# liuyuan-pal/NeuRay

Measured on AMD Instinct MI355X. Metric: rays/sec (64 coarse+32 fine samples), lego 800x800 synthetic, higher is better.
Workload: dtype fp32 (MLP contractions: operands split exactly into 3 bf16 parts, 6 bf16-MFMA products per K = 32, fp32 accumulate); 1 GPU; lego-800 synthetic (nerf_synthetic/lego/black_800 shape): 800x800 = 640000 rays/image, 8 ref views, 64 coarse + 32 fine samples, maps 200x200x32, 1 image per step per GPU; ray_batch=65536, parallelism=images sharded over 1 GPU(s), no collective

## Files before the change

### neuray_amd/csrc/nr_kernels.h

```cpp
#pragma once
#include "nr_device.h"

namespace nr {

__global__ void view_setup_kernel(const float* __restrict__ poses, const float* __restrict__ Ks,
                                  const float* __restrict__ depth_range, int n, float* __restrict__ out) {
    const int v = blockIdx.x * blockDim.x + threadIdx.x;
    if (v >= n) return;
    const float* P = poses + v * 12;
    const float* K = Ks + v * 9;
    float* o = out + v * kViewConst;
    for (int i = 0; i < 3; ++i)
        for (int j = 0; j < 4; ++j)
            o[i * 4 + j] = dot3(K[i * 3 + 0], K[i * 3 + 1], K[i * 3 + 2], P[j], P[4 + j], P[8 + j]);
    for (int i = 0; i < 3; ++i) o[12 + i] = dot3(-P[i], -P[4 + i], -P[8 + i], P[3], P[7], P[11]);
    o[15] = rn_div(-1.0f, depth_range[2 * v]);
    o[16] = rn_div(-1.0f, depth_range[2 * v + 1]);
    o[17] = rn_div(1.0f, rn_sub(o[16], o[15]));
    o[18] = 0.0f; o[19] = 0.0f;
}

__global__ void query_setup_kernel(const float* __restrict__ pose, const float* __restrict__ Kinv,
                                   const float* __restrict__ depth_range, float* __restrict__ o) {
    if (blockIdx.x * blockDim.x + threadIdx.x != 0) return;
    for (int i = 0; i < 9; ++i) o[i] = Kinv[i];
    for (int i = 0; i < 12; ++i) o[9 + i] = pose[i];
    for (int i = 0; i < 3; ++i) o[21 + i] = dot3(-pose[i], -pose[4 + i], -pose[8 + i], pose[3], pose[7], pose[11]);
    o[24] = rn_div(-1.0f, depth_range[0]);
    o[25] = rn_div(-1.0f, depth_range[1]);
    o[26] = depth_range[0];
    o[27] = rn_div(1.0f, rn_sub(o[25], o[24]));
}

__global__ void relayout_kernel(const float* __restrict__ src, float* __restrict__ dst, int n, int c, int h, int w, int c_pad) {
    const long long total = (long long)n * h * w;
    for (long long i = (long long)blockIdx.x * blockDim.x + threadIdx.x; i < total; i += (long long)gridDim.x * blockDim.x) {
        const long long img = i / ((long long)h * w);
        const long long pix = i - img * h * w;
        const float* s = src + img * c * h * w + pix;
        float* d = dst + i * c_pad;
        for (int ch = 0; ch < c_pad; ++ch) d[ch] = ch < c ? s[(long long)ch * h * w] : 0.0f;
    }
}

__global__ void coarse_depth_kernel(const float* __restrict__ depth_range, const float* __restrict__ rnd, int rn, int dn,
                                    float* __restrict__ out) {
    const float near = depth_range[0], far = depth_range[1];
    const long long total = (long long)rn * dn;
    for (long long i = (long long)blockIdx.x * blockDim.x + threadIdx.x; i < total; i += (long long)gridDim.x * blockDim.x) {
        const int k = (int)(i % dn);
        if (rnd && k > 0 && k < dn - 1) {
            const float inv_near = rn_div(1.0f, near);
            const float step = rn_div(rn_sub(rn_div(1.0f, far), inv_near), (float)(dn - 1));
            const float val = rn_add((float)k, rn_mul(rn_sub(rnd[(i / dn) * (dn - 2) + (k - 1)], 0.5f), 0.999f));
            out[i] = rn_div(1.0f, rn_add(inv_near, rn_mul(step, val)));
        } else {
            out[i] = coarse_depth(near, far, k, dn);
        }
    }
}

struct PointParams {
    const float* que_const;
    const float* view_const;
    const float* coords;
    const float* depth;
    const float* ray_feats;
    const float* img_feats;
    const float* rgba;
    const float* weights;
    float* point_out;
    float* dbg;
    float* saved;
    int rfn, rn, dn, h, w, fh, fw;
    int use_vis;
    float var_bias;
    int folded;
    unsigned long long* slot_stats;
};

constexpr int kDbgFields = 16;

constexpr int kSavedBgRow = 0, kSavedStatRow = 16, kSavedMsumRow = 60, kSavedSw0Row = 61, kSavedGeoRow = 62, kSavedGmeanRow = 78,
              kSavedGvarRow = 86, kSavedGRow = 94, kSavedZmaxRow = 98, kSavedSezRow = 99, kSavedSvisRow = 100, kSavedDist = 101 * 64;
constexpr int kSavedTileFloats = kSavedDist + 8 * 8 * 16;

__device__ __forceinline__ float sel4(int g, float a, float b, float c, float d) {
    return g == 0 ? a : (g == 1 ? b : (g == 2 ? c : d));
}

template <int NT>
constexpr int point_rmax() { return 12 * NT; }

template <int NT>
inline size_t point_smem_bytes(int nwaves, int ar = AR_F32) {
    return sizeof(float) * (64 * ((size_t)(nwaves + 1) * point_rmax<NT>() + (ar == AR_X3 ? 0 : 16 * NT)) + weight_lds_floats(ar));
}

template <int NT, int OWN, int STAT, class WS>
__device__ __forceinline__ void bg_accumulate(WS W, int lane, int g, int wave, int nw,
                                              const float (&st)[NT * 11], v4f (&accg)[OWN][NT]) {
    float xq[NT][8], x1[NT][1];
    NR_PRAGMA_UNROLL
    for (int t = 0; t < NT; ++t) {
        NR_PRAGMA_UNROLL
        for (int s = 0; s < 8; ++s) xq[t][s] = st[t * 11 + s];
        x1[t][0] = sel4(g, st[t * 11 + 8], st[t * 11 + 9], st[t * 11 + 10], 0.0f);
    }
    NR_PRAGMA_UNROLL
    for (int j = 0; j < OWN; ++j) {
        const int mo = wave + j * nw;
        if (mo < 4) layer_tile_slice<L_BG, NT, 2 * STAT, 2, STAT, 1>(W, lane, mo, xq, x1, accg[j]);
    }
}

template <int OWN> struct BgResident { float4 q[OWN][8]; float s1[OWN][4]; float4 b[OWN]; };
template <int OWN, class WS>
__device__ __forceinline__ void bg_resident_load(WS W, int lane, int wave, int nw, BgResident<OWN>& r) {
    constexpr int AR = ws_ar<WS>::value;
    NR_PRAGMA_UNROLL
    for (int j = 0; j < OWN; ++j) {
        const int mo = wave + j * nw, m = mo < 4 ? mo : 0;
        NR_PRAGMA_UNROLL
        for (int kq = 0; kq < 8; ++kq) r.q[j][kq] = wld4(W, lane * 16 + m * (8 * 1024), (quads_offset(L_BG, AR) + kq * 256) * 4);
        NR_PRAGMA_UNROLL
        for (int k1 = 0; k1 < 4; ++k1) r.s1[j][k1] = wld1(W, lane * 4 + m * (4 * 256), (single_offset(L_BG, AR) + k1 * 64) * 4);
        r.b[j] = wld4(W, (lane >> 4) * 16 + m * 64, bias_offset(L_BG, AR) * 4);
    }
}
template <int NT, int OWN, int STAT>
__device__ __forceinline__ void bg_accumulate(const BgResident<OWN>& r, int g, int wave, int nw,
                                              const float (&st)[NT * 11], v4f (&accg)[OWN][NT]) {
    float xq[NT][8], x1[NT][1];
    NR_PRAGMA_UNROLL
    for (int t = 0; t < NT; ++t) {
        NR_PRAGMA_UNROLL
        for (int s = 0; s < 8; ++s) xq[t][s] = st[t * 11 + s];
        x1[t][0] = sel4(g, st[t * 11 + 8], st[t * 11 + 9], st[t * 11 + 10], 0.0f);
    }
    NR_PRAGMA_UNROLL
    for (int j = 0; j < OWN; ++j) {
        const int mo = wave + j * nw;
        if (mo < 4) {
            mfma_quad<NT>(r.q[j][2 * STAT], 0, xq, accg[j]);
            mfma_quad<NT>(r.q[j][2 * STAT + 1], 1, xq, accg[j]);
            NR_PRAGMA_UNROLL
            for (int t = 0; t < NT; ++t) accg[j][t] = nr_mfma16(r.s1[j][STAT], x1[t][0], accg[j][t]);
        }
    }
}

template <int NA, int IDLE, int R, int RMAX, int OP>
__device__ __forceinline__ void view_allreduce(const float (&v)[NA > 0 ? NA : 1][R], float (&out)[R], float* red, int wave,
                                               int nw, int lane) {
    NR_PRAGMA_UNROLL
    for (int r = 0; r < R; ++r) {
        const bool is_max = OP == RED_MAX || (OP == RED_MAX0 && r == 0);
        float a = NA > 0 ? v[0][r] : (is_max ? -1e9f : 0.0f);
        NR_PRAGMA_UNROLL
        for (int s = 1; s < NA; ++s) a = red_combine<OP, R>(a, v[s][r], r);
        if (IDLE > 0 && NA > 0 && is_max) a = fmaxf(a, -1e9f);
        out[r] = a;
    }
    block_allreduce<R, RMAX, OP, R>(out, red, wave, nw, lane);
}

template <int N> struct SlotCount { static constexpr int value = N; };

#ifndef NR_POINT_SKIP
#define NR_POINT_SKIP 1
#endif
#ifndef NR_POINT_TILE_ORDER
#define NR_POINT_TILE_ORDER 0
#endif
#ifndef NR_POINT_TRANSPOSED
#define NR_POINT_TRANSPOSED 1
#endif

template <int NT, int VPW, bool HAS_VIS, int OWN, int MAXT, int MINW, bool SAVE = false, bool DBG = false, int AR = AR_F32>
__global__ void __launch_bounds__(MAXT, MINW) points_kernel(PointParams p) {
    static_assert(NT == 1, "one 16-point tile per wave iteration");
    static_assert(AR == AR_F32 || !SAVE, "the training forward runs on the fp32 MFMA");
    NR_DYNAMIC_SMEM(float, smem);
    constexpr int RMAX = point_rmax<NT>();
    constexpr int NS = VPW;
    constexpr bool SKIP = (NR_POINT_SKIP != 0) && !SAVE && !DBG && VPW == 2;
    const int lane = threadIdx.x & 63;
    const int wave = NR_UNIFORM((int)(threadIdx.x >> 6));
    const int nw = (p.rfn + VPW - 1) / VPW;
    const int g = lane >> 4, c = lane & 15;
    float* red = smem;
    float* xch = smem + (size_t)(nw + 1) * RMAX * 64;
    float* wl = xch + (AR == AR_X3 ? 0 : 16 * NT * 64);
    auto xrow = [&](int mo, int r) -> float* {
        if constexpr (AR == AR_X3 && OWN == 1) return red + ((size_t)mo * RMAX + r) * 64;
        else if constexpr (AR == AR_X3) return red + ((size_t)(mo % nw) * RMAX + (mo / nw) * 4 + r) * 64;
        else return xch + (mo * 4 + r) * 64;
    };
    auto make_w = [&]() {
        if constexpr (AR == AR_X3) return GlbW3{nr_make_wbuf(p.weights, sizeof(float) * kPackedPointFloatsX3)};
        else return nr_make_wbuf(p.weights, sizeof(float) * kPackedPassFloats);
    };
    const auto W = make_w();
    const float w_m1 = (float)(p.w - 1), h_m1 = (float)(p.h - 1);
    const float inv_w_m1 = 1.0f / w_m1, inv_h_m1 = 1.0f / h_m1, inv_rfn = 1.0f / (float)p.rfn;
    const size_t fmap = (size_t)p.fh * p.fw * 32, imap = (size_t)p.h * p.w * 4;
    const nr_mbuf rf_map = nr_make_mbuf(p.ray_feats, sizeof(float) * fmap * p.rfn);
    const nr_mbuf if_map = nr_make_mbuf(p.img_feats, sizeof(float) * fmap * p.rfn);
    const nr_mbuf rgb_map = nr_make_mbuf(p.rgba, sizeof(float) * imap * p.rfn);
    const int goff = 32 * g;
    const int npts = p.rn * p.dn;
    const int dn = p.dn;
    const bool use_vis = p.use_vis != 0;
    const bool folded = AR == AR_X3 || (!SAVE && p.folded != 0);
    const int bid = (int)(blockIdx.x % 8) * (int)(gridDim.x / 8) + (int)(blockIdx.x / 8);
    int seq0 = 0;
#ifndef NR_X3_BG_RESIDENT
#define NR_X3_BG_RESIDENT 1
#endif
#ifndef NR_X3_GF_PREFETCH
#define NR_X3_GF_PREFETCH 1
#endif
    constexpr bool BG_RES = AR == AR_X3 && OWN == 1 && (NR_X3_BG_RESIDENT != 0);
    BgResident<OWN> bgres;
    if constexpr (BG_RES) bg_resident_load(W, lane, wave, nw, bgres);
    int n_active = 0, n_slots = 0;
    constexpr bool TR = (NR_POINT_TRANSPOSED != 0) && !SAVE && !DBG;
    const int nloop = TR ? ((p.rn + 15) / 16) * dn * 16 : npts;
#ifndef NR_POINT_CHUNK
#define NR_POINT_CHUNK 1
#endif
    constexpr int CH = NR_POINT_CHUNK;
    const int G = (int)gridDim.x;
    auto tile_base = [&](int it) { return (((it / CH) * G + bid) * CH + (it % CH)) * 16; };
    if (tile_base(0) < nloop) stage_issue<PH_DIST_M>(wl, W, wave, nw, lane);
    for (int it = 0, base; (base = tile_base(it)) < nloop; ++it, seq0 += phase_count(HAS_VIS)) {
        const bool more = tile_base(it + 1) < nloop;
        const int glane = lane + nr_opaque_zero();
#ifndef NR_NO_OPAQUE_WAVE
        const int wave_t = wave + nr_opaque_szero();
#else
        const int wave_t = wave;
#endif
        const int gg = glane >> 4;
        const bool dbg_lane = DBG && (gg == 0);
        const auto* pt = NR_ARGS_HERE(PointParams, p);
        int pidx; bool pvalid;
        float mask[NS], dlt[NS][4], tref[NS], pu[NS], pv[NS], lo, hi;
        int soff_f[NS], soff_c[NS];
        {
            int pi, ray, smp;
            const float* __restrict__ qc = pt->que_const;
            const float qnearp = qc[24], qfarp = qc[25], qinv = qc[27];
            const int dn = pt->dn, npts = pt->rn * dn;
            if constexpr (TR) {
#if NR_POINT_TILE_ORDER == 1
                const int tix = base >> 4, nrb = (pt->rn + 15) / 16;
                smp = tix / nrb;
                const int rb = tix - smp * nrb;
#else
                const int tix = base >> 4, rb = tix / dn;
                smp = tix - rb * dn;
#endif
                ray = rb * 16 + c;
                pvalid = ray < pt->rn;
                ray = pvalid ? ray : pt->rn - 1;
                pi = ray * dn + smp;
            } else {
                pi = base + c;
                pvalid = pi < npts;
                pi = pi < npts ? pi : npts - 1;
                ray = pi / dn;
                smp = pi - ray * dn;
            }
            pidx = pi;
            const Ray r = make_ray<false>(qc, pt->coords[2 * ray], pt->coords[2 * ray + 1]);
            const float* drow = pt->depth + (size_t)ray * dn;
            const float d = drow[smp];
            float s_c, s_n, s_p, s_x;
            {
                const int nxt = smp + 1 < dn ? smp + 1 : smp, prv = smp > 0 ? smp - 1 : 0;
                const float dg = drow[gg == 0 ? smp : (gg == 1 ? nxt : prv)];
                nr_group_gather4(norm_inv_depth_fast(dg, qnearp, qfarp, qinv), s_c, s_n, s_p, s_x);
            }
            const float half_c = (smp == dn - 1) ? 500000.0f : (s_n - s_c) * 0.5f;
            const float half_p = (s_c - s_p) * 0.5f;
            hi = half_c;
            lo = (smp == 0) ? half_c : half_p;
            const float px = rn_add(r.cx, rn_mul(r.dx, d));
            const float py = rn_add(r.cy, rn_mul(r.dy, d));
            const float pz = rn_add(r.cz, rn_mul(r.dz, d));
            NR_PRAGMA_UNROLL
            for (int s = 0; s < NS; ++s) {
                const int vraw = wave_t * VPW + s;
                const bool vok = vraw < pt->rfn;
                const int view = vok ? vraw : pt->rfn - 1;
                const float* __restrict__ vc = pt->view_const + view * kViewConst;
                Proj pr = project_point<false>(vc, px, py, pz, (float)pt->w, (float)pt->h);
                if (!vok) pr.mask = 0.0f;
                mask[s] = pr.mask;
                dlt[s][0] = pr.dirx - r.qx; dlt[s][1] = pr.diry - r.qy; dlt[s][2] = pr.dirz - r.qz;
                dlt[s][3] = dot3(pr.dirx, pr.diry, pr.dirz, r.qx, r.qy, r.qz);
                tref[s] = norm_inv_depth_fast(fmaxf(pr.z, 1e-5f), vc[15], vc[16], vc[17]);
                pu[s] = pr.u; pv[s] = pr.v;
                if (dbg_lane && pvalid && vok) {
                    float* d_ = pt->dbg + ((size_t)pi * pt->rfn + view) * kDbgFields;
                    d_[0] = pr.mask; d_[1] = pr.u; d_[2] = pr.v; d_[3] = pr.z;
                }
                soff_f[s] = view * (int)(fmap * sizeof(float)); soff_c[s] = view * (int)(imap * sizeof(float));
            }
        }

        auto tile = [&](auto na_tag) NR_LAMBDA_INLINE {
            constexpr int NA = decltype(na_tag)::value, NA1 = NA > 0 ? NA : 1, IDLE = NS - NA;
            constexpr bool SC = NA == 2 && !SAVE;
            float fray[NA1][8], fimg[NA1][8], rgb[NA1][3];
#ifdef NR_PROBE_PRE
            float fm1[NA1][8], fv1[NA1][8], fa1[NA1][8];
#endif
            if constexpr (NA > 0) {
                Taps tfs[NA], tcs[NA];
                NR_PRAGMA_UNROLL
                for (int s = 0; s < NA; ++s) {
                    tfs[s] = make_taps_fast(pu[s], pv[s], w_m1, h_m1, inv_w_m1, inv_h_m1, p.fw, p.fh, p.fw == p.w && p.fh == p.h);
                    tcs[s] = make_taps_fast(pu[s], pv[s], w_m1, h_m1, inv_w_m1, inv_h_m1, p.w, p.h, true);
#ifdef NR_PROBE_NO_GATHER
                    tfs[s].o00 = tfs[s].o10 = tfs[s].o01 = tfs[s].o11 = 0;
                    tcs[s].o00 = tcs[s].o10 = tcs[s].o01 = tcs[s].o11 = 0;
#endif
                }
                NR_PRAGMA_UNROLL
                for (int s = 0; s < NA; ++s) {
                    float4 qf[8], qi[8], qc4[4];
                    issue8(rf_map, goff, soff_f[s], tfs[s], qf);
                    issue8(if_map, goff, soff_f[s], tfs[s], qi);
                    issue_rgb(rgb_map, soff_c[s], tcs[s], qc4);
                    NR_PIN();
                    blend8(qf, tfs[s], mask[s], fray[s]);
                    blend8(qi, tfs[s], mask[s], fimg[s]);
                    blend_rgb(qc4, tcs[s], mask[s], rgb[s]);
                    NR_PRAGMA_UNROLL
                    for (int k = 0; k < 8; ++k) { NR_KEEP(fray[s][k]); NR_KEEP(fimg[s][k]); }
                    NR_PRAGMA_UNROLL
                    for (int j = 0; j < 3; ++j) NR_KEEP(rgb[s][j]);
                    NR_PIN();
#ifdef NR_PROBE_PRE
                    {
                        float4 q1[8], q2[8], q3[8];
                        issue8(rf_map, goff, soff_f[s] + 4096, tfs[s], q1);
                        issue8(rf_map, goff, soff_f[s] + 8192, tfs[s], q2);
                        issue8(rf_map, goff, soff_f[s] + 12288, tfs[s], q3);
                        NR_PIN();
                        blend8(q1, tfs[s], mask[s], fm1[s]);
                        blend8(q2, tfs[s], mask[s], fv1[s]);
                        blend8(q3, tfs[s], mask[s], fa1[s]);
                        NR_PRAGMA_UNROLL
                        for (int k = 0; k < 8; ++k) { NR_KEEP(fm1[s][k]); NR_KEEP(fv1[s][k]); NR_KEEP(fa1[s][k]); }
                        NR_PIN();
                    }
#endif
                }
            }
            float none[NA1][1];
            NR_PRAGMA_UNROLL
            for (int s = 0; s < NA1; ++s) none[s][0] = 0.0f;
// ... 215 lines not shown
                        p12[s][11] = mask[s];
                    }
                    view_allreduce<NA, IDLE, 12, RMAX, RED_SUM>(p12, o12, red, wave_t, nw, lane);
                    msum = o12[11];
                    const float inv = nr_fast_rcp(msum + 1e-8f);
                    NR_PRAGMA_UNROLL
                    for (int q = 0; q < 11; ++q) st[q] = o12[q] * inv;
                    NR_PRAGMA_UNROLL
                    for (int s = 0; s < NA; ++s) wv[s] = mask[s] * nr_fast_rcp(msum + 1e-8f);
                    if constexpr (SAVE) {
                        if (wave_t == 0) p.saved[(size_t)(base / 16) * kSavedTileFloats + kSavedMsumRow * 64 + lane] = msum;
                    }
                }
                NR_PRAGMA_UNROLL
                for (int k = 0; k < 2; ++k) {
                    NR_PRAGMA_UNROLL
                    for (int s = 0; s < NA; ++s) wk[s] = k == 0 ? sn[s] * wv[s] : wv[s];
                    if (k == 1) {
                        NR_PRAGMA_UNROLL
                        for (int s = 0; s < NA; ++s) {
                            NR_PRAGMA_UNROLL
                            for (int q = 0; q < 8; ++q) part[s][q] = gi[s][q] * wk[s];
                            NR_PRAGMA_UNROLL
                            for (int j = 0; j < 3; ++j) part[s][8 + j] = gr[s][j] * wk[s];
                        }
                        view_allreduce<NA, IDLE, 11, RMAX, RED_SUM>(part, st, red, wave_t, nw, lane);
                    }
                    NR_PRAGMA_UNROLL
                    for (int s = 0; s < NA; ++s) {
                        NR_PRAGMA_UNROLL
                        for (int q = 0; q < 8; ++q) { const float d_ = gi[s][q] - st[q]; part[s][q] = wk[s] * (d_ * d_); }
                        NR_PRAGMA_UNROLL
                        for (int j = 0; j < 3; ++j) { const float d_ = gr[s][j] - st[8 + j]; part[s][8 + j] = wk[s] * (d_ * d_); }
                    }
                    if constexpr (BG_RES) {
                        if (k == 0) bg_accumulate<NT, OWN, 0>(bgres, gg, wave_t, nw, st, accg);
                        else bg_accumulate<NT, OWN, 2>(bgres, gg, wave_t, nw, st, accg);
                    } else {
                        if (k == 0) bg_accumulate<NT, OWN, 0>(W, glane, gg, wave_t, nw, st, accg);
                        else bg_accumulate<NT, OWN, 2>(W, glane, gg, wave_t, nw, st, accg);
                    }
                    view_allreduce<NA, IDLE, 11, RMAX, RED_SUM>(part, sv, red, wave_t, nw, lane);
                    if constexpr (BG_RES) {
                        if (k == 0) bg_accumulate<NT, OWN, 1>(bgres, gg, wave_t, nw, sv, accg);
                        else bg_accumulate<NT, OWN, 3>(bgres, gg, wave_t, nw, sv, accg);
                    } else {
                        if (k == 0) bg_accumulate<NT, OWN, 1>(W, glane, gg, wave_t, nw, sv, accg);
                        else bg_accumulate<NT, OWN, 3>(W, glane, gg, wave_t, nw, sv, accg);
                    }
                    if constexpr (SAVE) {
                        float* d_ = p.saved + (size_t)(base / 16) * kSavedTileFloats + (kSavedStatRow + 22 * k) * 64 + lane;
                        if (wave_t == (2 * k) % nw) {
                            NR_PRAGMA_UNROLL
                            for (int q = 0; q < 11; ++q) d_[q * 64] = st[q];
                        }
                        if (wave_t == (2 * k + 1) % nw) {
                            NR_PRAGMA_UNROLL
                            for (int q = 0; q < 11; ++q) d_[(11 + q) * 64] = sv[q];
                        }
                    }
                }
                NR_PRAGMA_UNROLL
                for (int j = 0; j < OWN; ++j) {
                    const int mo = wave_t + j * nw;
                    if (mo < 4) {
                        NR_PRAGMA_UNROLL
                        for (int r = 0; r < 4; ++r) xrow(mo, r)[lane] = accg[j][0][r];
                        if constexpr (SAVE) {
                            NR_PRAGMA_UNROLL
                            for (int r = 0; r < 4; ++r)
                                p.saved[(size_t)(base / 16) * kSavedTileFloats + (kSavedBgRow + mo * 4 + r) * 64 + lane] = accg[j][0][r];
                        }
                    }
                }
                NR_BLOCK_SYNC();
                NR_PRAGMA_UNROLL
                for (int s = 0; s < NA; ++s)
                    NR_PRAGMA_UNROLL
                    for (int mo = 0; mo < (AR == AR_X3 ? 2 : 4); ++mo)
                        NR_PRAGMA_UNROLL
                        for (int r = 0; r < 4; ++r) accv[s][mo][r] = xrow(mo, r)[lane];
            }
            float x[NA1][8], vis2[NA1], z[NA1];
            constexpr bool GF_PRE = BG_RES && (NR_X3_GF_PREFETCH != 0);
            float4 gfq[4]; float gfs = 0.0f;
            typename ws_lds<decltype(make_w())>::type W5;
            LayerPreT<L_VF1, AR> p_vf1;
            {
                float xq[NA1][16], x1[NA1][1], h64[NA1][16];
                Opnd3<NA1, 16> xq3;
                LayerPreT<L_BV0, AR> p_bv0; LayerPreT<L_BV1, AR> p_bv1; LayerPreT<L_B2, AR> p_b2;
                v4f acch[NA1][2];
                if constexpr (NA > 0) {
                    NR_PRAGMA_UNROLL
                    for (int s = 0; s < NA; ++s) {
                        NR_PRAGMA_UNROLL
                        for (int k = 0; k < 8; ++k) { xq[s][k] = gi[s][k]; xq[s][8 + k] = e[s][k]; }
                        x1[s][0] = sel4(gg, gr[s][0], gr[s][1], gr[s][2], 0.0f);
                    }
                    layer_prefetch<L_BV0>(W4, lane, p_bv0);
                    NR_PRAGMA_UNROLL
                    for (int s = 0; s < NA; ++s) { acch[s][0] = accv[s][0]; acch[s][1] = accv[s][1]; }
                    if constexpr (AR == AR_X3) {
                        const Opnd3<NA1, 8> gi3 = split_operand(gi);
                        NR_PRAGMA_UNROLL
                        for (int pt = 0; pt < 3; ++pt)
                            NR_PRAGMA_UNROLL
                            for (int s = 0; s < NA; ++s)
                                NR_PRAGMA_UNROLL
                                for (int i = 0; i < 4; ++i) { xq3.p[pt][s][i] = gi3.p[pt][s][i]; xq3.p[pt][s][4 + i] = e3.p[pt][s][i]; }
                        layer_acc<L_BV0, NA>(W4, lane, p_bv0, xq3, x1, acch, last);
                    } else layer_acc<L_BV0, NA>(W4, lane, p_bv0, xq, x1, acch, last);
                    NR_PRAGMA_UNROLL
                    for (int s = 0; s < NA; ++s)
                        NR_PRAGMA_UNROLL
                        for (int mo = 0; mo < 2; ++mo)
                            NR_PRAGMA_UNROLL
                            for (int r = 0; r < 4; ++r) h64[s][4 * mo + r] = elu_s(acch[s][mo][r]);
                }
                const auto W4b = phase_enter<PH_BV1, HAS_VIS>(wl, W, seq0, true, wave_t, nw, lane);
                if constexpr (NA > 0) {
                    layer_prefetch<L_BV1>(W4b, lane, p_bv1);
                    NR_PRAGMA_UNROLL
                    for (int s = 0; s < NA; ++s) {
                        if constexpr (AR == AR_X3) {
                            NR_PRAGMA_UNROLL
                            for (int mo = 0; mo < 2; ++mo)
                                NR_PRAGMA_UNROLL
                                for (int r = 0; r < 4; ++r) acch[s][mo][r] = xrow(2 + mo, r)[lane];
                        } else { acch[s][0] = accv[s][2]; acch[s][1] = accv[s][3]; }
                    }
                    if constexpr (AR == AR_X3) layer_acc<L_BV1, NA>(W4b, lane, p_bv1, xq3, x1, acch, last);
                    else layer_acc<L_BV1, NA>(W4b, lane, p_bv1, xq, x1, acch, last);
                    NR_PRAGMA_UNROLL
                    for (int s = 0; s < NA; ++s)
                        NR_PRAGMA_UNROLL
                        for (int mo = 0; mo < 2; ++mo)
                            NR_PRAGMA_UNROLL
                            for (int r = 0; r < 4; ++r) h64[s][8 + 4 * mo + r] = elu_s(acch[s][mo][r]);
                }
                W5 = phase_enter<PH_B2_VF1, HAS_VIS>(wl, W, seq0, true, wave_t, nw, lane);
                if constexpr (NA > 0) {
                    layer_prefetch<L_B2>(W5, lane, p_b2);
                    layer_fwd<L_B2, NA, ACT_ELU>(W5, lane, p_b2, operand<AR>(h64), none, x, p_vf1);
                }
            }
            {
                float xin[NA1][8], h[NA1][8];
                if constexpr (NA > 0) {
                    NR_PRAGMA_UNROLL
                    for (int s = 0; s < NA; ++s)
                        NR_PRAGMA_UNROLL
                        for (int k = 0; k < 8; ++k) xin[s][k] = x[s][k] * wv[s];
                    layer_fwd<L_VF1, NA, ACT_ELU>(W5, lane, p_vf1, operand<AR>(xin), none, h, last);
                }
                W5 = phase_enter<PH_TAIL, HAS_VIS>(wl, W, seq0, more, wave_t, nw, lane);
                if constexpr (GF_PRE) {
                    const int m = wave_t < 4 ? wave_t : 0;
                    NR_PRAGMA_UNROLL
                    for (int kq = 0; kq < 4; ++kq) gfq[kq] = wld4(W, glane * 16 + m * (4 * 1024), (quads_offset(L_GF1, AR) + kq * 256) * 4);
                    gfs = wld1(W, glane * 4 + m * 256, single_offset(L_GF1, AR) * 4);
                }
                if constexpr (NA > 0) {
                    float y[NA][8], yv[NA][1], o[NA][1];
                    LayerPreT<L_VF2, AR> p_vf2; LayerPreT<L_V21, AR> p_v21; LayerPreT<L_RF1, AR> p_rf1; LayerPreT<L_RF2, AR> p_rf2;
                    VecPre<L_VF2> p_vf2v; VecPre<L_V22> p_v22; VecPre<L_RF3> p_rf3;
                    layer_prefetch<L_VF2>(W5, lane, p_vf2);
                    layer_prefetch<L_VF2>(W5, lane, p_vf2v);
                    layer_fwd<L_VF2, NA, ACT_ELU>(W5, lane, p_vf2, operand<AR>(h), none, y, p_v21);
                    if constexpr (SC) nr_group_gather2(sigmoidf(elu(layer_vec_scatter_1x2<L_VF2, 0>(p_vf2v, h))), yv[0][0], yv[1][0]);
                    else {
                        layer_vec<L_VF2, NA>(p_vf2v, h, yv);
                        NR_PRAGMA_UNROLL
                        for (int s = 0; s < NA; ++s) yv[s][0] = sigmoidf(elu(yv[s][0]));
                    }
                    float visp[NA];
                    NR_PRAGMA_UNROLL
                    for (int s = 0; s < NA; ++s) {
                        visp[s] = yv[s][0] * mask[s];
                        NR_PRAGMA_UNROLL
                        for (int k = 0; k < 8; ++k) { x[s][k] = x[s][k] + y[s][k]; xin[s][k] = x[s][k] * visp[s]; }
                    }
                    Opnd3<NA, 8> x3;
                    if constexpr (AR == AR_X3) {
                        x3 = split_operand(x);
                        layer_fwd_scaled<L_V21, NA, ACT_ELU>(W5, lane, p_v21, x3, visp, h, p_v22);
                    } else layer_fwd<L_V21, NA, ACT_ELU>(W5, lane, p_v21, xin, none, h, p_v22);
                    layer_prefetch<L_RF1>(W5, lane, p_rf1);
                    if constexpr (SC) nr_group_gather2(sigmoidf(layer_vec_scatter_1x2<L_V22, 0>(p_v22, h)), o[0][0], o[1][0]);
                    else {
                        layer_vec<L_V22, NA>(p_v22, h, o);
                        NR_PRAGMA_UNROLL
                        for (int s = 0; s < NA; ++s) o[s][0] = sigmoidf(o[s][0]);
                    }
                    NR_PRAGMA_UNROLL
                    for (int s = 0; s < NA; ++s) vis2[s] = o[s][0] * mask[s];
                    float x1[NA][2], h16[NA][4], h8[NA][4];
                    NR_PRAGMA_UNROLL
                    for (int s = 0; s < NA; ++s) {
                        x1[s][0] = sel4(gg, vis2[s], dlt[s][0], dlt[s][1], dlt[s][2]);
                        x1[s][1] = sel4(gg, dlt[s][3], 0.0f, 0.0f, 0.0f);
                    }
                    if constexpr (AR == AR_X3) layer_fwd<L_RF1, NA, ACT_ELU>(W5, lane, p_rf1, x3, x1, h16, p_rf2);
                    else layer_fwd<L_RF1, NA, ACT_ELU>(W5, lane, p_rf1, x, x1, h16, p_rf2);
                    layer_fwd<L_RF2, NA, ACT_ELU>(W5, lane, p_rf2, operand<AR>(h16), none, h8, p_rf3);
                    if constexpr (SC) nr_group_gather2(layer_vec_scatter_1x2<L_RF3, 0>(p_rf3, h8), o[0][0], o[1][0]);
                    else layer_vec<L_RF3, NA>(p_rf3, h8, o);
                    NR_PRAGMA_UNROLL
                    for (int s = 0; s < NA; ++s) {
                        z[s] = mask[s] > 0.0f ? o[s][0] : -1e9f;
                        const int vraw = wave_t * VPW + s;
                        if (dbg_lane && pvalid && vraw < p.rfn) {
                            float* d_ = pt->dbg + ((size_t)pidx * pt->rfn + vraw) * kDbgFields;
                            d_[12] = sn[s]; d_[13] = visp[s]; d_[14] = vis2[s]; d_[15] = z[s];
                        }
                    }
                }
            }
            constexpr int ZR = SAVE ? 3 : 2;
            float zv[ZR], big[12], wh[NA1], meanw;
            {
                float z2[NA1][ZR];
                NR_PRAGMA_UNROLL
                for (int s = 0; s < NA; ++s) {
                    z2[s][0] = z[s]; z2[s][1] = vis2[s];
                    if constexpr (SAVE) z2[s][2] = sn[s] * wv[s];
                }
                view_allreduce<NA, IDLE, ZR, RMAX, RED_MAX0>(z2, zv, red, wave_t, nw, lane);
                float b12[NA1][12];
                NR_PRAGMA_UNROLL
                for (int s = 0; s < NA; ++s) {
                    const float ev = nr_fast_exp(z[s] - zv[0]);
                    wh[s] = vis2[s] * nr_fast_rcp(zv[1] + 1e-8f);
                    NR_PRAGMA_UNROLL
                    for (int k = 0; k < 8; ++k) b12[s][k] = x[s][k] * wh[s];
                    b12[s][8] = ev;
                    NR_PRAGMA_UNROLL
                    for (int j = 0; j < 3; ++j) b12[s][9 + j] = rgb[s][j] * ev;
                }
                if constexpr (IDLE > 0) {
                    const float ev_idle = nr_fast_exp(-1e9f - zv[0]);
                    if constexpr (NA == 0) {
                        NR_PRAGMA_UNROLL
                        for (int q = 0; q < 12; ++q) b12[0][q] = 0.0f;
                        float acc_ = ev_idle;
                        NR_PRAGMA_UNROLL
                        for (int i = 1; i < IDLE; ++i) acc_ += ev_idle;
                        b12[0][8] = acc_;
                        view_allreduce<1, 0, 12, RMAX, RED_SUM>(b12, big, red, wave_t, nw, lane);
                    } else {
                        NR_PRAGMA_UNROLL
                        for (int i = 0; i < IDLE; ++i) b12[NA - 1][8] += ev_idle;
                        view_allreduce<NA, 0, 12, RMAX, RED_SUM>(b12, big, red, wave_t, nw, lane);
                    }
                } else {
                    view_allreduce<NA, 0, 12, RMAX, RED_SUM>(b12, big, red, wave_t, nw, lane);
                }
                {
                    const float ie = nr_fast_rcp(big[8]);
                    big[9] *= ie; big[10] *= ie; big[11] *= ie;
                    meanw = zv[1] * nr_fast_rcp(zv[1] + 1e-8f);
                }
                if constexpr (SAVE) {
                    float* d_ = p.saved + (size_t)(base / 16) * kSavedTileFloats + lane;
                    if (wave_t == 0) {
                        NR_PRAGMA_UNROLL
                        for (int k = 0; k < 8; ++k) d_[(kSavedGmeanRow + k) * 64] = big[k];
                    }
                    if (wave_t == 2 % nw) {
                        d_[kSavedZmaxRow * 64] = zv[0]; d_[kSavedSezRow * 64] = big[8];
                        d_[kSavedSvisRow * 64] = zv[1]; d_[kSavedSw0Row * 64] = zv[ZR - 1];
                    }
                }
            }
            v4f accf[OWN][1];
            NR_PRAGMA_UNROLL
            for (int j = 0; j < OWN; ++j) {
                const int mo = wave_t + j * nw;
                const float4 b = wld4(W, gg * 16 + (mo < 4 ? mo : 0) * 64, bias_offset(L_GF1, AR) * 4);
                accf[j][0][0] = b.x; accf[j][0][1] = b.y; accf[j][0][2] = b.z; accf[j][0][3] = b.w;
            }
            float var[8];
            {
                float xq[1][8], x1[1][1], v8[NA1][8];
                NR_PRAGMA_UNROLL
                for (int s = 0; s < NA; ++s)
                    NR_PRAGMA_UNROLL
                    for (int k = 0; k < 8; ++k) { const float d_ = x[s][k] - big[k]; v8[s][k] = wh[s] * (d_ * d_); }
                NR_PRAGMA_UNROLL
                for (int k = 0; k < 8; ++k) xq[0][k] = big[k];
                x1[0][0] = sel4(gg, meanw * inv_rfn, 0.0f, 0.0f, 0.0f);
                NR_PRAGMA_UNROLL
                for (int j = 0; j < OWN; ++j) {
                    const int mo = wave_t + j * nw;
                    if constexpr (GF_PRE) {
                        if (mo < 4) {
                            mfma_quad<NT>(gfq[0], 0, xq, accf[j]);
                            mfma_quad<NT>(gfq[1], 1, xq, accf[j]);
                            accf[j][0] = nr_mfma16(gfs, x1[0][0], accf[j][0]);
                        }
                    } else if (mo < 4) layer_tile_slice<L_GF1, NT, 0, 2, 0, 1>(W, glane, mo, xq, x1, accf[j]);
                }
                view_allreduce<NA, IDLE, 8, RMAX, RED_SUM>(v8, var, red, wave_t, nw, lane);
                if constexpr (SAVE) {
                    if (wave_t == 1 % nw) {
                        NR_PRAGMA_UNROLL
                        for (int k = 0; k < 8; ++k) p.saved[(size_t)(base / 16) * kSavedTileFloats + (kSavedGvarRow + k) * 64 + lane] = var[k];
                    }
                }
            }
            {
                float xq[1][8], nonet[1][1];
                nonet[0][0] = 0.0f;
                NR_PRAGMA_UNROLL
                for (int k = 0; k < 8; ++k) xq[0][k] = var[k];
                NR_PRAGMA_UNROLL
                for (int j = 0; j < OWN; ++j) {
                    const int mo = wave_t + j * nw;
                    if (mo < 4) {
                        if constexpr (GF_PRE) { mfma_quad<NT>(gfq[2], 0, xq, accf[j]); mfma_quad<NT>(gfq[3], 1, xq, accf[j]); }
                        else layer_tile_slice<L_GF1, NT, 2, 2, 0, 0>(W, glane, mo, xq, nonet, accf[j]);
                        NR_PRAGMA_UNROLL
                        for (int r = 0; r < 4; ++r) xrow(mo, r)[lane] = elu_s(accf[j][0][r]);
                        if constexpr (SAVE) {
                            NR_PRAGMA_UNROLL
                            for (int r = 0; r < 4; ++r)
                                p.saved[(size_t)(base / 16) * kSavedTileFloats + (kSavedGeoRow + mo * 4 + r) * 64 + lane] = elu_s(accf[j][0][r]);
                        }
                    }
                }
            }
            NR_BLOCK_SYNC();
            if (wave_t == 0) {
                float h[1][16], G[1][4], nonet[1][1];
                nonet[0][0] = 0.0f;
                NR_PRAGMA_UNROLL
                for (int k = 0; k < 16; ++k) h[0][k] = xrow(k >> 2, k & 3)[lane];
                layer_fwd<L_GF2, NT, ACT_ELU>(W, glane, h, nonet, G);
                if (pvalid)
                    *reinterpret_cast<float4*>(pt->point_out + (size_t)pidx * kPointRec + 4 * g) = make_float4(G[0][0], G[0][1], G[0][2], G[0][3]);
                if constexpr (SAVE) {
                    NR_PRAGMA_UNROLL
                    for (int r = 0; r < 4; ++r) p.saved[(size_t)(base / 16) * kSavedTileFloats + (kSavedGRow + r) * 64 + lane] = G[0][r];
                }
            }
            if (wave_t == (nw > 1 ? 1 : 0) && gg == 0) {
                if (pvalid)
                    *reinterpret_cast<float4*>(pt->point_out + (size_t)pidx * kPointRec + 16) = make_float4(big[9], big[10], big[11], msum);
            }
        };

        if constexpr (SKIP) {
            const bool a0 = __ballot(mask[0] != 0.0f) != 0ull, a1 = __ballot(mask[1] != 0.0f) != 0ull;
#ifdef NR_FORCE_NA
#ifdef NR_FORCE_NA_CONST
            const int na = NR_FORCE_NA;
#else
            const int na = NR_FORCE_NA + (p.rn < 0 ? (a0 ? 1 : 0) + (a1 ? 1 : 0) : 0);
#endif
#else
            const int na = (a0 ? 1 : 0) + (a1 ? 1 : 0);
#endif
            n_active += na; n_slots += NS;
            if (na == 2) {
                tile(SlotCount<2>{});
            } else if (na == 1) {
                if (!a0) {
                    mask[0] = mask[1]; tref[0] = tref[1]; pu[0] = pu[1]; pv[0] = pv[1]; soff_f[0] = soff_f[1]; soff_c[0] = soff_c[1];
                    NR_PRAGMA_UNROLL
                    for (int k = 0; k < 4; ++k) dlt[0][k] = dlt[1][k];
                }
                tile(SlotCount<1>{});
            } else {
                tile(SlotCount<0>{});
            }
        } else {
            tile(SlotCount<NS>{});
        }
    }
    if constexpr (SKIP) {
        if (p.slot_stats) {
            NR_BLOCK_SYNC();
            if (lane == 0) { red[2 * wave] = (float)n_active; red[2 * wave + 1] = (float)n_slots; }
            NR_BLOCK_SYNC();
            if (threadIdx.x == 0) {
                float a = 0.0f, b = 0.0f;
                for (int w = 0; w < nw; ++w) { a += red[2 * w]; b += red[2 * w + 1]; }
                atomicAdd(p.slot_stats, (unsigned long long)a);
                atomicAdd(p.slot_stats + 1, (unsigned long long)b);
            }
        }
    }
}

struct RayParams {
    const float* point_rec;
    const float* depth;
    const float* pos_enc;
    const float* weights;
    float* hit_prob;
    float* pixel;
    float* render_depth;
    unsigned char* ray_mask;
    float* density;
    float* att_save;
    int rn, dn, mask_view_num, mask_point_num;
};
constexpr int kRayAttSave = 24;

constexpr int kRayWaves = 4;
inline size_t ray_smem_bytes(int dn, int rays_per_wave = 1) { return sizeof(float) * (kPackedRayFloats + 12 + kRayWaves * rays_per_wave * ((size_t)dn * 34)); }

__device__ __forceinline__ float wave_sum(float v) {
    NR_PRAGMA_UNROLL
    for (int m = 32; m >= 1; m >>= 1) v += __shfl_xor(v, m);
    return v;
}

__device__ __forceinline__ float wave_max(float v) {
    NR_PRAGMA_UNROLL
    for (int m = 32; m >= 1; m >>= 1) v = fmaxf(v, __shfl_xor(v, m));
// ... 685 lines not shown
```

### neuray_amd/csrc/nr_layout.h

```cpp
#pragma once

namespace nr {

enum LayerId {
    L_DM1, L_DM2,
    L_DFIN_M,
    L_DV1, L_DV2,
    L_DFIN_V,
    L_DA1, L_DA2,
    L_DFIN_A,
    L_DS1, L_DS2,
    L_DFIN_S,
    L_PE1, L_PE2,
    L_RD1, L_RD2,
    L_NF1, L_NF2,
    L_BV0, L_BV1,
    L_B2,
    L_VF1, L_VF2,
    L_V21, L_V22,
    L_RF1, L_RF2, L_RF3,
    L_BG,
    L_GF1, L_GF2,
    L_FWD_COUNT,
    LT_DM1 = L_FWD_COUNT, LT_DM2, LT_DV1, LT_DV2, LT_DA1, LT_DA2, LT_DS1, LT_DS2,
// ... 57 lines not shown
};

struct VecShape { int n, tiles; };
constexpr VecShape kVec[L_COUNT] = {
    {0, 0}, {0, 0}, {2, 2},
    {0, 0}, {0, 0}, {2, 2},
    {0, 0}, {0, 0}, {1, 2},
    {0, 0}, {0, 0}, {1, 2},
    {0, 0}, {0, 0},
    {0, 0}, {3, 1},
    {0, 0}, {1, 1},
    {0, 0}, {0, 0}, {0, 0},
    {0, 0}, {1, 2},
    {0, 0}, {1, 2},
    {0, 0}, {0, 0}, {1, 1},
    {0, 0},
    {0, 0}, {0, 0},
    {0, 0}, {0, 0}, {0, 0}, {0, 0}, {0, 0}, {0, 0}, {0, 0}, {0, 0},
    {2, 2}, {0, 0},
    {0, 0},
    {0, 0},
    {3, 4},
    {0, 0},
    {0, 0},
    {3, 4}, {3, 4}, {3, 4}, {3, 4},
    {0, 0}, {0, 0},
    {0, 0},
    {1, 1}, {0, 0},
    {1, 4}, {0, 0},
};

constexpr int AR_F32 = 0, AR_X3 = 1;
constexpr bool ar_omits(int l, int ar) { return ar == AR_X3 && l == L_PE2; }
constexpr bool ar_splits(int l, int ar) { return ar == AR_X3 && l != L_BG && l != L_GF1 && l != L_GF2; }

constexpr int quads_floats(int l, int ar = AR_F32) { return ar_omits(l, ar) ? 0 : kShape[l].mt_out * kShape[l].kq * 64 * (ar_splits(l, ar) ? 6 : 4); }
constexpr int single_floats(int l, int ar = AR_F32) { return ar_omits(l, ar) ? 0 : kShape[l].mt_out * kShape[l].k1 * 64; }
constexpr int bias_floats(int l, int ar = AR_F32) { return ar_omits(l, ar) ? 0 : kShape[l].mt_out * 16; }
constexpr int vec_floats(int l, int ar = AR_F32) { return (kVec[l].n > 0 && !ar_omits(l, ar)) ? kVec[l].n * kVec[l].tiles * 16 + 16 : 0; }
constexpr int layer_floats(int l, int ar = AR_F32) { return quads_floats(l, ar) + single_floats(l, ar) + bias_floats(l, ar) + vec_floats(l, ar); }
constexpr int tile_quads_floats(int l, int ar = AR_F32) { return kShape[l].kq * 64 * (ar_splits(l, ar) ? 6 : 4); }

constexpr int layer_offset(int l, int ar = AR_F32) {
    int off = 0;
    for (int i = (l >= L_FWD_COUNT ? (int)L_FWD_COUNT : 0); i < l; ++i) off += layer_floats(i, ar);
    return off;
}
constexpr int quads_offset(int l, int ar = AR_F32) { return layer_offset(l, ar); }
constexpr int single_offset(int l, int ar = AR_F32) { return layer_offset(l, ar) + quads_floats(l, ar); }
constexpr int bias_offset(int l, int ar = AR_F32) { return layer_offset(l, ar) + quads_floats(l, ar) + single_floats(l, ar); }
constexpr int vec_offset(int l, int ar = AR_F32) { return bias_offset(l, ar) + bias_floats(l, ar); }
constexpr int vec_bias_offset(int l, int ar = AR_F32) { return vec_offset(l, ar) + kVec[l].n * kVec[l].tiles * 16; }

constexpr int packed_range_floats(int first, int last, int ar = AR_F32) {
    int off = 0;
    for (int i = first; i < last; ++i) off += layer_floats(i, ar);
    return off;
}
constexpr int kPackedPointFloats = packed_range_floats(0, L_FWD_COUNT);
constexpr int kPackedPointFloatsX3 = packed_range_floats(0, L_FWD_COUNT, AR_X3);
constexpr int kPackedTFloats = packed_range_floats(L_FWD_COUNT, L_COUNT);

enum PhaseId { PH_DIST_M, PH_DIST_VA, PH_DIST_S, PH_EMBED, PH_NF_BV0, PH_BV1, PH_B2_VF1, PH_TAIL, PH_COUNT };
struct PhaseRange { int first, last; };
constexpr PhaseRange kPhase[PH_COUNT] = {
    {L_DM1, L_DV1},
    {L_DV2, L_DFIN_A},
    {L_DS1, L_DFIN_S},
    {L_PE1, L_RD2},
    {L_NF1, L_BV0},
    {L_BV1, L_BV1},
    {L_B2, L_VF1},
    {L_VF2, L_RF3},
};
constexpr int phase_begin(int ph, int ar = AR_F32) { return layer_offset(kPhase[ph].first, ar); }
constexpr int phase_floats(int ph, int ar = AR_F32) { return layer_offset(kPhase[ph].last + 1, ar) - layer_offset(kPhase[ph].first, ar); }
constexpr int max_phase_floats(int ar = AR_F32) {
    int m = 0;
    for (int i = 0; i < PH_COUNT; ++i) m = phase_floats(i, ar) > m ? phase_floats(i, ar) : m;
    return m;
}
constexpr int stage_region_bytes(int ar = AR_F32) { return (max_phase_floats(ar) * 4 + 1023) / 1024 * 1024; }
constexpr int weight_lds_floats(int ar = AR_F32) { return 2 * stage_region_bytes(ar) / 4; }
constexpr int kStageRegionBytes = stage_region_bytes();
constexpr int kWeightLdsFloats = weight_lds_floats();
constexpr int phase_count(bool vis) { return vis ? PH_COUNT : PH_COUNT - 1; }
constexpr int phase_seq(int ph, bool vis) { return (vis || ph < PH_DIST_S) ? ph : ph - 1; }
constexpr int phase_next(int ph, bool vis) {
    return ph == PH_COUNT - 1 ? 0 : ((!vis && ph + 1 == PH_DIST_S) ? ph + 2 : ph + 1);
}

constexpr int RW_WQ = 0, RW_WK = 256, RW_WV = 512, RW_FC = 768, RW_LNW = 1024, RW_LNB = 1040,
              RW_OG0W = 1056, RW_OG0B = 1312, RW_OG2W = 1328, RW_OG2B = 1344, kPackedRayFloats = 1348;

constexpr int kPackedPassFloats = kPackedPointFloats + kPackedRayFloats;

constexpr int kPointRec = 20;

constexpr int kViewConst = 20;
constexpr int kMaxViews = 16;
constexpr int kQueryConst = 28;

enum PassTensor {
    T_MEAN0_W, T_MEAN0_B, T_MEAN2_W, T_MEAN2_B, T_MEAN4_W, T_MEAN4_B,
    T_VAR0_W, T_VAR0_B, T_VAR2_W, T_VAR2_B, T_VAR4_W, T_VAR4_B,
    T_AW0_W, T_AW0_B, T_AW2_W, T_AW2_B, T_AW4_W, T_AW4_B,
    T_VIS0_W, T_VIS0_B, T_VIS2_W, T_VIS2_B, T_VIS4_W, T_VIS4_B,
    T_PE0_W, T_PE0_B, T_PE2_W, T_PE2_B,
    T_RD0_W, T_RD0_B, T_RD2_W, T_RD2_B,
    T_BASE0_W, T_BASE0_B, T_BASE2_W, T_BASE2_B,
    T_VF0_W, T_VF0_B, T_VF2_W, T_VF2_B,
    T_V20_W, T_V20_B, T_V22_W, T_V22_B,
    T_GF0_W, T_GF0_B, T_GF2_W, T_GF2_B,
    T_WQ, T_WK, T_WV, T_FC, T_LN_W, T_LN_B,
    T_OG0_W, T_OG0_B, T_OG2_W, T_OG2_B,
    T_RF0_W, T_RF0_B, T_RF2_W, T_RF2_B, T_RF4_W, T_RF4_B,
    T_NF0_W, T_NF0_B, T_NF2_W, T_NF2_B,
    T_COUNT
};

constexpr int kTensorRows[T_COUNT] = {
    32, 32, 32, 32, 2, 2,   32, 32, 32, 32, 2, 2,   32, 32, 32, 32, 1, 1,   32, 32, 32, 32, 1, 1,
    32, 32, 32, 32,   16, 16, 35, 35,   64, 64, 32, 32,   32, 32, 33, 33,   32, 32, 1, 1,   64, 64, 16, 16,
    16, 16, 16, 16, 16, 16,   16, 16, 1, 1,   16, 16, 8, 8, 1, 1,   8, 8, 1, 1,
};
constexpr int kTensorCols[T_COUNT] = {
    32, 1, 32, 1, 32, 1,   32, 1, 32, 1, 32, 1,   32, 1, 32, 1, 32, 1,   32, 1, 32, 1, 32, 1,
    34, 1, 32, 1,   4, 1, 16, 1,   207, 1, 64, 1,   32, 1, 32, 1,   32, 1, 32, 1,   65, 1, 64, 1,
    16, 16, 16, 16, 1, 1,   16, 1, 16, 1,   37, 1, 16, 1, 8, 1,   32, 1, 8, 1,
};
constexpr int tensor_floats(int t) { return kTensorRows[t] * kTensorCols[t]; }
constexpr int tensor_offset(int t) {
    int off = 0;
    for (int i = 0; i < t; ++i) off += tensor_floats(i);
    return off;
}
constexpr int kFlatPassFloats = tensor_offset(T_COUNT);

}
```

Baseline: 3.346 million rays/s.

## Stage geometry_fc weights in LDS and prefetch next tile's ray inputs

```diff
diff --git a/neuray_amd/csrc/nr_kernels.h b/neuray_amd/csrc/nr_kernels.h
--- a/neuray_amd/csrc/nr_kernels.h
+++ b/neuray_amd/csrc/nr_kernels.h
@@ -92,9 +92,11 @@
 template <int NT>
 constexpr int point_rmax() { return 12 * NT; }
 
+inline bool point_gf_lds(int nwaves, int ar) { return ar == AR_X3 && nwaves >= 4; }
 template <int NT>
 inline size_t point_smem_bytes(int nwaves, int ar = AR_F32) {
-    return sizeof(float) * (64 * ((size_t)(nwaves + 1) * point_rmax<NT>() + (ar == AR_X3 ? 0 : 16 * NT)) + weight_lds_floats(ar));
+    return sizeof(float) * (64 * ((size_t)(nwaves + 1) * point_rmax<NT>() + (ar == AR_X3 ? 0 : 16 * NT)) + weight_lds_floats(ar) +
+                            (point_gf_lds(nwaves, ar) ? gf_lds_floats(ar) : 0));
 }
 
 template <int NT, int OWN, int STAT, class WS>
@@ -218,9 +220,6 @@
 #ifndef NR_X3_BG_RESIDENT
 #define NR_X3_BG_RESIDENT 1
 #endif
-#ifndef NR_X3_GF_PREFETCH
-#define NR_X3_GF_PREFETCH 1
-#endif
     constexpr bool BG_RES = AR == AR_X3 && OWN == 1 && (NR_X3_BG_RESIDENT != 0);
     BgResident<OWN> bgres;
     if constexpr (BG_RES) bg_resident_load(W, lane, wave, nw, bgres);
@@ -233,7 +232,40 @@
     constexpr int CH = NR_POINT_CHUNK;
     const int G = (int)gridDim.x;
     auto tile_base = [&](int it) { return (((it / CH) * G + bid) * CH + (it % CH)) * 16; };
-    if (tile_base(0) < nloop) stage_issue<PH_DIST_M>(wl, W, wave, nw, lane);
+#ifndef NR_POINT_CARRY_F32
+#define NR_POINT_CARRY_F32 0
+#endif
+    constexpr bool CARRY = TR && OWN == 1 && (AR == AR_X3 || (NR_POINT_CARRY_F32 != 0));
+    float in_x = 0.0f, in_y = 0.0f, in_d = 0.0f, in_dg = 0.0f;
+    auto tile_inputs = [&](const auto* pt, int tbase, int gg) {
+        const int dn = pt->dn, tix = tbase >> 4;
+#if NR_POINT_TILE_ORDER == 1
+        const int nrb = (pt->rn + 15) / 16, smp = tix / nrb, rb = tix - smp * nrb;
+#else
+        const int rb = tix / dn, smp = tix - rb * dn;
+#endif
+        int ray = rb * 16 + c;
+        ray = ray < pt->rn ? ray : pt->rn - 1;
+        const float* drow = pt->depth + (size_t)ray * dn;
+        const int nxt = smp + 1 < dn ? smp + 1 : smp, prv = smp > 0 ? smp - 1 : 0;
+        in_x = pt->coords[2 * ray]; in_y = pt->coords[2 * ray + 1];
+        in_d = drow[smp];
+        in_dg = drow[gg == 0 ? smp : (gg == 1 ? nxt : prv)];
+    };
+    constexpr bool GF_LDS = AR == AR_X3 && OWN == 1;
+    auto make_wg = [&]() {
+        if constexpr (GF_LDS) return typename ws_lds<decltype(make_w())>::type{wl + weight_lds_floats(AR), gf_lds_begin(AR) * 4};
+        else return W;
+    };
+    const auto WG = make_wg();
+    if (tile_base(0) < nloop) {
+        stage_issue<PH_DIST_M>(wl, W, wave, nw, lane);
+        if constexpr (GF_LDS) {
+            for (int c_ = wave; c_ < gf_lds_floats(AR) / 256; c_ += nw)
+                nr_dma16(ws_raw(W), wl + weight_lds_floats(AR) + c_ * 256, lane, lane * 16, gf_lds_begin(AR) * 4 + c_ * 1024);
+        }
+        if constexpr (CARRY) tile_inputs(NR_ARGS_HERE(PointParams, p), tile_base(0), g);
+    }
     for (int it = 0, base; (base = tile_base(it)) < nloop; ++it, seq0 += phase_count(HAS_VIS)) {
         const bool more = tile_base(it + 1) < nloop;
         const int glane = lane + nr_opaque_zero();
@@ -274,13 +306,13 @@
                 smp = pi - ray * dn;
             }
             pidx = pi;
-            const Ray r = make_ray<false>(qc, pt->coords[2 * ray], pt->coords[2 * ray + 1]);
+            const Ray r = make_ray<false>(qc, CARRY ? in_x : pt->coords[2 * ray], CARRY ? in_y : pt->coords[2 * ray + 1]);
             const float* drow = pt->depth + (size_t)ray * dn;
-            const float d = drow[smp];
+            const float d = CARRY ? in_d : drow[smp];
             float s_c, s_n, s_p, s_x;
             {
                 const int nxt = smp + 1 < dn ? smp + 1 : smp, prv = smp > 0 ? smp - 1 : 0;
-                const float dg = drow[gg == 0 ? smp : (gg == 1 ? nxt : prv)];
+                const float dg = CARRY ? in_dg : drow[gg == 0 ? smp : (gg == 1 ? nxt : prv)];
                 nr_group_gather4(norm_inv_depth_fast(dg, qnearp, qfarp, qinv), s_c, s_n, s_p, s_x);
             }
             const float half_c = (smp == dn - 1) ? 500000.0f : (s_n - s_c) * 0.5f;
@@ -662,8 +694,6 @@
                         for (int r = 0; r < 4; ++r) accv[s][mo][r] = xrow(mo, r)[lane];
             }
             float x[NA1][8], vis2[NA1], z[NA1];
-            constexpr bool GF_PRE = BG_RES && (NR_X3_GF_PREFETCH != 0);
-            float4 gfq[4]; float gfs = 0.0f;
             typename ws_lds<decltype(make_w())>::type W5;
             LayerPreT<L_VF1, AR> p_vf1;
             {
@@ -735,11 +765,8 @@
                     layer_fwd<L_VF1, NA, ACT_ELU>(W5, lane, p_vf1, operand<AR>(xin), none, h, last);
                 }
                 W5 = phase_enter<PH_TAIL, HAS_VIS>(wl, W, seq0, more, wave_t, nw, lane);
-                if constexpr (GF_PRE) {
-                    const int m = wave_t < 4 ? wave_t : 0;
-                    NR_PRAGMA_UNROLL
-                    for (int kq = 0; kq < 4; ++kq) gfq[kq] = wld4(W, glane * 16 + m * (4 * 1024), (quads_offset(L_GF1, AR) + kq * 256) * 4);
-                    gfs = wld1(W, glane * 4 + m * 256, single_offset(L_GF1, AR) * 4);
+                if constexpr (CARRY) {
+                    if (more) tile_inputs(pt, tile_base(it + 1), gg);
                 }
                 if constexpr (NA > 0) {
                     float y[NA][8], yv[NA][1], o[NA][1];
@@ -857,7 +884,7 @@
             NR_PRAGMA_UNROLL
             for (int j = 0; j < OWN; ++j) {
                 const int mo = wave_t + j * nw;
-                const float4 b = wld4(W, gg * 16 + (mo < 4 ? mo : 0) * 64, bias_offset(L_GF1, AR) * 4);
+                const float4 b = wld4(WG, gg * 16 + (mo < 4 ? mo : 0) * 64, bias_offset(L_GF1, AR) * 4);
                 accf[j][0][0] = b.x; accf[j][0][1] = b.y; accf[j][0][2] = b.z; accf[j][0][3] = b.w;
             }
             float var[8];
@@ -873,13 +900,7 @@
                 NR_PRAGMA_UNROLL
                 for (int j = 0; j < OWN; ++j) {
                     const int mo = wave_t + j * nw;
-                    if constexpr (GF_PRE) {
-                        if (mo < 4) {
-                            mfma_quad<NT>(gfq[0], 0, xq, accf[j]);
-                            mfma_quad<NT>(gfq[1], 1, xq, accf[j]);
-                            accf[j][0] = nr_mfma16(gfs, x1[0][0], accf[j][0]);
-                        }
-                    } else if (mo < 4) layer_tile_slice<L_GF1, NT, 0, 2, 0, 1>(W, glane, mo, xq, x1, accf[j]);
+                    if (mo < 4) layer_tile_slice<L_GF1, NT, 0, 2, 0, 1>(WG, glane, mo, xq, x1, accf[j]);
                 }
                 view_allreduce<NA, IDLE, 8, RMAX, RED_SUM>(v8, var, red, wave_t, nw, lane);
                 if constexpr (SAVE) {
@@ -898,8 +919,7 @@
                 for (int j = 0; j < OWN; ++j) {
                     const int mo = wave_t + j * nw;
                     if (mo < 4) {
-                        if constexpr (GF_PRE) { mfma_quad<NT>(gfq[2], 0, xq, accf[j]); mfma_quad<NT>(gfq[3], 1, xq, accf[j]); }
-                        else layer_tile_slice<L_GF1, NT, 2, 2, 0, 0>(W, glane, mo, xq, nonet, accf[j]);
+                        layer_tile_slice<L_GF1, NT, 2, 2, 0, 0>(WG, glane, mo, xq, nonet, accf[j]);
                         NR_PRAGMA_UNROLL
                         for (int r = 0; r < 4; ++r) xrow(mo, r)[lane] = elu_s(accf[j][0][r]);
                         if constexpr (SAVE) {
@@ -916,7 +936,7 @@
                 nonet[0][0] = 0.0f;
                 NR_PRAGMA_UNROLL
                 for (int k = 0; k < 16; ++k) h[0][k] = xrow(k >> 2, k & 3)[lane];
-                layer_fwd<L_GF2, NT, ACT_ELU>(W, glane, h, nonet, G);
+                layer_fwd<L_GF2, NT, ACT_ELU>(WG, glane, h, nonet, G);
                 if (pvalid)
                     *reinterpret_cast<float4*>(pt->point_out + (size_t)pidx * kPointRec + 4 * g) = make_float4(G[0][0], G[0][1], G[0][2], G[0][3]);
                 if constexpr (SAVE) {
diff --git a/neuray_amd/csrc/nr_layout.h b/neuray_amd/csrc/nr_layout.h
--- a/neuray_amd/csrc/nr_layout.h
+++ b/neuray_amd/csrc/nr_layout.h
@@ -163,6 +163,9 @@
 }
 constexpr int stage_region_bytes(int ar = AR_F32) { return (max_phase_floats(ar) * 4 + 1023) / 1024 * 1024; }
 constexpr int weight_lds_floats(int ar = AR_F32) { return 2 * stage_region_bytes(ar) / 4; }
+constexpr int gf_lds_begin(int ar) { return layer_offset(L_GF1, ar); }
+constexpr int gf_lds_floats(int ar) { return ((layer_floats(L_GF1, ar) + layer_floats(L_GF2, ar)) * 4 + 1023) / 1024 * 256; }
+static_assert(L_GF2 == L_GF1 + 1 && L_GF2 + 1 == L_FWD_COUNT, "geometry_fc's layers are one contiguous range of the packed buffer");
 constexpr int kStageRegionBytes = stage_region_bytes();
 constexpr int kWeightLdsFloats = weight_lds_floats();
 constexpr int phase_count(bool vis) { return vis ? PH_COUNT : PH_COUNT - 1; }
```

After: 1.700 million rays/s. 0.508x the previous value.
